# DataZooDE/anofox-forecast

Measured on AMD Instinct MI355X. Metric: series/sec fit+forecast, AutoETS h=28 on M5-shape batches, higher is better.
Workload: dtype f64

## Files before the change

anofox-forecast_amd/csrc/host_api.hip:

```cpp
#include <hip/hip_runtime.h>

#include <algorithm>
#include <cctype>
#include <atomic>
#include <memory>
#include <unordered_map>
#include <chrono>
#include <cmath>
#include <condition_variable>
#include <mutex>
#include <cstdio>
#include <cstdlib>
#include <cstring>
#include <limits>
#include <map>
#include <stdexcept>
#include <string>
#include <system_error>
#include <thread>
#include <vector>

#include "classic_device.hpp"
#include "host_semantics.hpp"
#include "kernels.hpp"
// ... 68 lines not shown
    int32_t *d_count = nullptr;
    int32_t *d_pos_map = nullptr, *d_pos_cnt = nullptr, *d_notpos = nullptr;
    double *d_ypos = nullptr;
    bool use_pos = false;
    bool none_pos = false;
    std::vector<anofox::FitArgs> insp_args;
    std::vector<anofox::FitLaunchers> insp_fns;
    std::vector<int> insp_spec, insp_stream;
    bool insp_ok = false;
    int insp_m = 1;
    int32_t live_pos = -1, live_all = -1;
    int arima_method = 0;
    size_t ar_ws_bytes = 0;
    double *ar_w = nullptr, *ar_wmean = nullptr, *ar_wsd = nullptr, *ar_l0 = nullptr, *ar_l1 = nullptr, *ar_x = nullptr, *ar_aicc = nullptr;
    int32_t *ar_wlen = nullptr, *ar_d = nullptr, *ar_D = nullptr, *ar_order = nullptr, *ar_status = nullptr, *ar_evals = nullptr, *ar_passes = nullptr, *ar_models = nullptr;
    StreamSet *sset = nullptr;
    hipStream_t own_stream = nullptr;
    hipStream_t aux[N_AUX_STREAMS] = {};
    hipEvent_t ev_start = nullptr, ev_stop = nullptr, ev_fit0 = nullptr, ev_fit1 = nullptr, ev_fork = nullptr;
    hipEvent_t ev_join[N_AUX_STREAMS] = {};
    struct Lane {
        double *ybuf = nullptr;
        size_t ybuf_cols = 0;
        int32_t *map[2] = {nullptr, nullptr};
        int32_t *cnt = nullptr;
        anofox::NmStateBuf st{};
        double *nm_scratch = nullptr;
        size_t nm_scratch_doubles = 0;
    } lanes[N_AUX_STREAMS];
    anofox::FitArgs *d_group_tab = nullptr, *h_group_tab = nullptr;
    size_t group_tab_cap = 0;
    hipEvent_t ev_group_tab = nullptr;
    hipStream_t last_stream = nullptr;
    bool ran = false, timed_fit = false;
    uint32_t fit_launches = 0;
    uint64_t n_problems = 0;
    Tunables tun;
    int seq_rounds = 3;
    int seq_rounds_env = -1;
    int spec_below_md = 8192;
    anofox::NmStateBuf classic_st{};
    int32_t *d_classic_status = nullptr, *classic_map[2] = {nullptr, nullptr}, *classic_cnt = nullptr;
    double *d_classic_ybuf = nullptr;
    size_t classic_ybuf_cols = 0;
    std::vector<void *> retired;
    int merged_m_max = 0;
    int32_t *d_m_col = nullptr;
    int spec2_below_md = 2048;
    int spec2_below = 1024;
    int spec_below = 8192;
    bool use_gather = false;
    double gather_budget = 0.0;
// ... 144 lines not shown
    if (b->owns_y) F(b->d_y);
    pin_free(b->h_stage);
    if (b->owns_len) F(b->d_len);
    F(b->d_mean); F(b->d_sd); F(b->d_fig_add); F(b->d_fig_mul); F(b->d_l0); F(b->d_b0); F(b->d_flags);
    F(b->d_aicc); F(b->d_yhat_slots); F(b->d_status_slots); F(b->d_evals_slots); F(b->d_iters_slots);
    F(b->d_passes_slots); F(b->d_slot_spec); F(b->d_lane_stats); F(b->d_wave_trace); F(b->d_yc32); F(b->d_yc16); F(b->d_misfit);
    F(b->d_yhat); F(b->d_lo); F(b->d_hi); F(b->d_model_code); F(b->d_status); F(b->d_detail);
    F(b->classic_st.sim); F(b->classic_st.fs); F(b->classic_st.phase); F(b->classic_st.evals); F(b->classic_st.iters); F(b->classic_st.passes); F(b->classic_st.done);
    F(b->d_classic_ybuf); F(b->d_classic_status); F(b->classic_map[0]); F(b->classic_map[1]); F(b->classic_cnt);
    for (void *p : b->retired) F(p);
    b->retired.clear();
    F(b->d_m_col); F(b->d_ring); F(b->d_prep_scratch);
    F(b->d_group_tab); pin_free(b->h_group_tab); b->d_group_tab = b->h_group_tab = nullptr; b->group_tab_cap = 0;
    if (b->ev_group_tab) { (void)hipEventDestroy(b->ev_group_tab); b->ev_group_tab = nullptr; }
    F(b->d_im_level); F(b->d_im_gmax); F(b->d_im_fc);
    F(b->d_th_sidx); F(b->d_th_adj);
    if (b->owns_exog) { F((void *)b->d_exog_x); F((void *)b->d_exog_f); }
    b->d_exog_x = b->d_exog_f = nullptr; b->owns_exog = false; b->exog_k = 0;
    F(b->d_exog_b0); F(b->d_exog_beta); F(b->d_exog_used);
    F(b->d_passes_total); F(b->d_evals_total); F(b->d_mask); F(b->d_len_group); F(b->d_count); F(b->d_pos_map); F(b->d_pos_cnt); F(b->d_notpos); F(b->d_ypos);
    F(b->ar_w); F(b->ar_wmean); F(b->ar_wsd); F(b->ar_l0); F(b->ar_l1); F(b->ar_x); F(b->ar_aicc); F(b->ar_wlen); F(b->ar_d); F(b->ar_D);
    F(b->ar_order); F(b->ar_status); F(b->ar_evals); F(b->ar_passes); F(b->ar_models);
    batch_detach_streams(b);
    for (auto &l : b->lanes) {
        F(l.ybuf); l.ybuf_cols = 0; F(l.map[0]); F(l.map[1]); F(l.cnt);
        F(l.st.sim); F(l.st.fs); F(l.st.phase); F(l.st.evals); F(l.st.iters); F(l.st.passes); F(l.st.done);
        F(l.nm_scratch); l.nm_scratch_doubles = 0;
    }
}

int max_slots_for(const Plan &p)
{
    if (p.model == M_AutoETS) return 30;
    if (p.model == M_ETS && p.ets_spec_id >= 0) return 1;
    return 0;
}

void alloc_common(AnofoxHipBatch *b)
{
    const size_t n = b->n, ld = b->ld, h = (size_t)std::max(b->h, 0);
    b->d_mean = dalloc<double>(ld);
    b->d_sd = dalloc<double>(ld);
    b->d_flags = dalloc<uint32_t>(ld);
    b->d_yhat = dalloc<double>(n * h);
    b->d_lo = dalloc<double>(n * h);
    b->d_hi = dalloc<double>(n * h);
    b->d_model_code = dalloc<int32_t>(ld);
    b->d_status = dalloc<int32_t>(ld);
// ... 22 lines not shown
        b->ar_status = dalloc<int32_t>(ld); b->ar_evals = dalloc<int32_t>(ld); b->ar_passes = dalloc<int32_t>(ld); b->ar_models = dalloc<int32_t>(ld);
        HIPCHECK(hipMemset(b->ar_wlen, 0, ld * sizeof(int32_t)));
    }
    HIPCHECK(hipMemset(b->d_model_code, 0, ld * sizeof(int32_t)));
    HIPCHECK(hipMemset(b->d_detail, 0, ld * sizeof(int32_t)));
    HIPCHECK(hipMemset(b->d_passes_total, 0, ld * sizeof(int32_t)));
    HIPCHECK(hipMemset(b->d_evals_total, 0, ld * sizeof(int32_t)));
    HIPCHECK(hipMemset(b->d_mask, 0, ld * sizeof(uint32_t)));
    b->n_slots_cap = max_slots_for(b->plan);
    if (b->n_slots_cap > 0) {
        const size_t S = (size_t)b->n_slots_cap;
        b->d_l0 = dalloc<double>(9 * ld);
        b->d_b0 = dalloc<double>(9 * ld);
        b->d_aicc = dalloc<double>(S * ld);
        b->d_yhat_slots = dalloc<double>(S * n * h);
        b->d_status_slots = dalloc<int32_t>(S * ld);
        b->d_evals_slots = dalloc<int32_t>(S * ld);
        b->d_iters_slots = dalloc<int32_t>(S * ld);
        b->d_passes_slots = dalloc<int32_t>(S * ld);
        b->d_slot_spec = dalloc<int32_t>(S);
        b->d_lane_stats = dalloc<unsigned long long>(2 * S);
        HIPCHECK(hipMemset(b->d_lane_stats, 0, 2 * S * sizeof(unsigned long long)));
        const int n_lanes = std::min<int>(N_AUX_STREAMS, b->n_slots_cap);
        for (int q = 0; q < n_lanes; q++) {
            auto &l = b->lanes[q];
            l.map[0] = dalloc<int32_t>(ld);
            l.map[1] = dalloc<int32_t>(ld);
            l.cnt = dalloc<int32_t>(3);
            l.st.sim = dalloc<double>(20 * ld);
            l.st.fs = dalloc<double>(5 * ld);
            l.st.phase = dalloc<int32_t>(ld);
            l.st.evals = dalloc<int32_t>(ld);
            l.st.iters = dalloc<int32_t>(ld);
            l.st.passes = dalloc<int32_t>(ld);
            l.st.done = dalloc<int32_t>(ld);
        }
    }
    batch_attach_streams(b);
}

void ensure_fig(AnofoxHipBatch *b, int m)
{
    if (m <= b->fig_m) return;
    if (b->d_fig_add) b->retired.push_back(b->d_fig_add);
    if (b->d_fig_mul) b->retired.push_back(b->d_fig_mul);
    b->d_fig_add = nullptr; b->d_fig_mul = nullptr; b->fig_m = 0;
    b->d_fig_add = dalloc<double>((size_t)m * b->ld);
    b->d_fig_mul = dalloc<double>((size_t)m * b->ld);
    b->fig_m = m;
}

// ... 146 lines not shown

void run_classic(AnofoxHipBatch *b, int kind, const int32_t *d_len, int m, int optimized, double alpha, int min_len,
                 const uint32_t *mask, uint32_t want, int32_t code, bool write_code, hipStream_t st)
{
    ClassicArgs a{};
    a.y = b->d_y; a.ld = b->ld; a.len = d_len; a.n_series = (int)b->n;
    a.m = m; a.h = b->h; a.optimized = optimized; a.fixed_alpha = alpha;
    a.mask = mask; a.want = want; a.min_len = min_len;
    a.yhat = b->d_yhat; a.status = b->d_detail; a.passes = b->d_passes_total;
    a.model_code = code; a.model_code_out = write_code ? b->d_model_code : nullptr;
    a.ring_scratch = nullptr;
    a.m_col = (kind == CK_HW || kind == CK_SEASONAL_ES) ? b->d_m_col : nullptr;
    const bool optimise = kind == CK_HOLT || kind == CK_HW || optimized != 0;
    if (optimise) {
        const size_t n = b->n, ld = b->ld;
        if (!b->classic_st.sim) {
            b->classic_st.sim = dalloc<double>(12 * ld); b->classic_st.fs = dalloc<double>(4 * ld);
            b->classic_st.phase = dalloc<int32_t>(ld); b->classic_st.evals = dalloc<int32_t>(ld); b->classic_st.iters = dalloc<int32_t>(ld);
            b->classic_st.passes = dalloc<int32_t>(ld); b->classic_st.done = dalloc<int32_t>(ld);
            b->d_classic_status = dalloc<int32_t>(ld);
            b->classic_map[0] = dalloc<int32_t>(ld); b->classic_map[1] = dalloc<int32_t>(ld); b->classic_cnt = dalloc<int32_t>(3);
        }
        double *ybuf = (b->n_slots_cap > 0 && b->use_gather) ? b->lanes[0].ybuf : nullptr;
        size_t ybuf_cols = ybuf ? b->lanes[0].ybuf_cols : ld;
        if (!ybuf) {
            const double per_col = (double)std::max<size_t>(b->t_max, 1) * 8.0;
            const size_t cols = (size_t)std::min((double)ld, 32.0 * 1073741824.0 / per_col) / 64 * 64;
            if (cols >= 1024 || cols >= ld) {
                if (!b->d_classic_ybuf) { b->d_classic_ybuf = dalloc<double>(std::max<size_t>(b->t_max, 1) * cols); b->classic_ybuf_cols = cols; }
                ybuf = b->d_classic_ybuf;
                ybuf_cols = b->classic_ybuf_cols;
            }
        }
        const bool seasonal = kind == CK_HW || kind == CK_SEASONAL_ES;
        FitArgs f{};
        f.y = b->d_y; f.ld = ld; f.len = d_len; f.n_series = (int)n; f.t_rows = (int)std::max<size_t>(b->t_max, 1);
        f.m = seasonal ? std::max(m, 1) : 1; f.h = b->h;
        f.flags = b->d_flags; f.fig = nullptr; f.fig_ld = ld;
        f.status = b->d_classic_status; f.st = b->classic_st;
        f.mask = mask; f.want = want; f.min_len = min_len;
        f.m_col = a.m_col;
        const bool merged = f.m_col != nullptr;
        FitLaunchers fns = classic_fit_launcher(kind, (merged && f.m == 7) ? 8 : f.m);
        if (!fns.round_seq || !fns.round_spec || !fns.round_spec2 || !fns.round_auto) throw HipFail{"no round kernel for this model"};
        if (f.m > ETS_LDS_PERIOD) {
            const size_t wg = merged ? n : std::max<size_t>((n + 15) / 16, std::min<size_t>(n, 1024));
            f.ring_scratch = ensure_ring(b, wg * (size_t)f.m * 64u);
// ... 319 lines not shown
            live_of[oi] = (spec_has_mult(specs[order[oi]]) && b->live_pos >= 0) ? (int64_t)b->live_pos : (b->live_all >= 0 ? (int64_t)b->live_all : (int64_t)n);
            lanes += live_of[oi];
        }
        const int64_t resident = 2 * 1024 * 64;
        const bool tiny_batch = (uint64_t)n * order.size() <= (uint64_t)TINY_BATCH_PROBLEMS;
        fill_mode = b->tun.fill_policy > 0 && !tiny_batch && !b->fixed_params && order.size() > 1 && b->seq_rounds_env < 0 && b->seq_rounds == 0 &&
                    lanes * 4 > 8 * resident;
        if (fill_mode) {
            const int64_t target = resident * (int64_t)b->tun.fill_target / 100;
            for (size_t oi = 0; oi < order.size(); oi++) {
                if (dead[oi] || k4[oi]) continue;
                if (lanes + 3 * live_of[oi] <= target) { fill_spec4[oi] = 1; lanes += 3 * live_of[oi]; }
            }
        }
    }
    if (b->use_gather && !b->fixed_params) {
        const size_t T = std::max<size_t>(b->t_max, 1);
        std::vector<size_t> need(order.size(), 0);
        double total = 0.0;
        for (size_t oi = 0; oi < order.size(); oi++) {
            if (dead[oi]) continue;
            size_t c = (b->use_pos && args[oi].need_positive && b->live_pos >= 0) ? (size_t)b->live_pos : n;
            need[oi] = std::min(ld, (c + 63) / 64 * 64);
            total += (double)need[oi] * (double)T * 8.0;
        }
        const double scale = total > b->gather_budget ? b->gather_budget / total : 1.0;
        for (size_t oi = 0; oi < order.size(); oi++) {
            if (dead[oi]) continue;
            auto &lane = b->lanes[oi % (size_t)n_lanes];
            size_t cols = scale < 1.0 ? (size_t)((double)need[oi] * scale) / 64 * 64 : need[oi];
            if (b->tun.gather_cols > 0) cols = std::min<size_t>(need[oi], (size_t)b->tun.gather_cols / 64 * 64);
            if (cols < need[oi] && cols < 1024 && b->tun.gather_cols <= 0) cols = 0;
            if (lane.ybuf && lane.ybuf_cols >= cols) continue;
            if (lane.ybuf) {
                HIPCHECK(hipDeviceSynchronize());
                dev_free(lane.ybuf, true);
                lane.ybuf = nullptr; lane.ybuf_cols = 0;
            }
            while (cols >= 64) {
                try { lane.ybuf = dalloc<double>(T * cols); lane.ybuf_cols = cols; break; }
                catch (const HipFail &f) {
                    if (!f.oom) throw;
                    cols = cols / 2 / 64 * 64;
                    if (cols < 1024) cols = 0;
                }
            }
        }
    }
    const bool tiny = (uint64_t)n * order.size() <= (uint64_t)TINY_BATCH_PROBLEMS;
    const int total_rounds = b->fixed_params ? 0 : (tiny ? 1 : n_rounds);
    enum { RK_SEQ, RK_SPEC, RK_SPEC2, RK_AUTO, RK_K4, RK_AUTO_K4 };
    std::vector<int> group_of(order.size(), -1);
    std::vector<std::vector<size_t>> groups;
    std::vector<int> group_stream;
    std::vector<GroupLaunchFn> group_fn;
    std::vector<size_t> slot_of(order.size(), 0);
    size_t n_slots = 0;
    bool grouped = b->tun.group_launch > 0 && !inline_stream && !tiny && !merged && !b->fixed_params && total_rounds > 0;
    if (grouped) {
        GroupLaunchFn fn[N_GROUP_CLASSES];
        for (int c = 0; c < N_GROUP_CLASSES; c++) fn[c] = ets_group_launcher(c, m, yt);
        std::vector<size_t> of_class[N_GROUP_CLASSES];
        for (size_t oi = 0; oi < order.size() && grouped; oi++) {
// ... 17 lines not shown
                }
                add(half[0], c); add(half[1], c);
            };
            if (b->tun.group_split == 1) add_split(of_class[GROUP_DAMPED_MUL], GROUP_DAMPED_MUL);
            else add(of_class[GROUP_DAMPED_MUL], GROUP_DAMPED_MUL);
            if (b->tun.group_split == 2) add_split(of_class[GROUP_GENERAL], GROUP_GENERAL);
            else add(of_class[GROUP_GENERAL], GROUP_GENERAL);
            add(of_class[GROUP_ADDITIVE], GROUP_ADDITIVE);
            grouped = !groups.empty();
        }
        if (grouped) {
            for (size_t g = 0; g < groups.size(); g++) {
                const bool dm = spec_trend_idx(specs[order[groups[g][0]]]) == 4;
                group_stream.push_back(dm ? (int)g : N_AUX_STREAMS - 1 - (int)g);
                for (size_t oi : groups[g]) { group_of[oi] = (int)g; stream_of[oi] = group_stream[g]; slot_of[oi] = n_slots++; }
            }
            for (size_t oi = 0; oi < order.size(); oi++) if (dead[oi]) stream_of[oi] = group_stream[0];
        }
    }
    bool emit = true;
    std::vector<int> slot_blocks, slot_k4;
    GroupCompactArgs gc{};
    GroupGatherArgs gg{};
    int gg_cols = 0;
    auto run_round = [&](const size_t oi, const int kind, const FitArgs &a, hipStream_t sq, const int r) {
        if (!grouped) {
            const FitLaunchFn f = kind == RK_SEQ ? fns[oi].round_seq : kind == RK_SPEC ? fns[oi].round_spec : kind == RK_SPEC2 ? fns[oi].round_spec2 :
                                  kind == RK_AUTO ? fns[oi].round_auto : kind == RK_K4 ? fns[oi].round_k4 : fns[oi].round_auto_k4;
            f(a, sq);
            return;
        }
        if (emit) return;
        FitArgs t = a;
        if (kind == RK_SEQ || kind == RK_K4) { t.spec_below = -1; t.spec2_below = -1; t.budget_seq = t.budget; }
        else if (kind == RK_SPEC) { t.spec_below = 0x7fffffff; t.spec2_below = -1; }
        else if (kind == RK_SPEC2) throw HipFail{"launch_fit_slots: the one-wave-per-problem round of a tiny batch has no group form"};
        const int g_seq = (int)((n + NM_BLOCK - 1) / NM_BLOCK);
        const int g_spec = (int)((std::min<int64_t>((int64_t)n, std::max(t.spec_below, 0)) + NM_BLOCK / NM_K - 1) / (NM_BLOCK / NM_K));
        const int g_spec2 = (int)std::min<int64_t>((int64_t)n, std::max(t.spec2_below, 0));
        const int blocks = std::max(g_seq, std::max(g_spec, g_spec2));
        if (t.ring_scratch != nullptr && (size_t)blocks * (size_t)t.m * NM_BLOCK > t.ring_scratch_doubles)
            throw HipFail{"launch_fit_slots: the seasonal-ring scratch does not cover a group slot"};
        const size_t cell = (size_t)r * n_slots + slot_of[oi];
        b->h_group_tab[cell] = t;
        slot_blocks[cell] = blocks;
        slot_k4[cell] = (kind == RK_K4 || kind == RK_AUTO_K4) ? 1 : 0;
// ... 11 lines not shown
            a.spec_below = -1; a.spec2_below = -1;
            a.gathered = 0;
            if (tiny) {
                a.y_round = b->d_y; a.ld_round = ld; a.series_of = nullptr; a.n_active = nullptr;
                a.budget = 1 << 30; a.budget_seq = a.budget;
                run_round(oi, RK_SPEC2, a, sq, r);
                b->fit_launches++;
                return;
            }
            if (r == 0 && b->use_pos && a.need_positive) {
                if (emit)
                    hipLaunchKernelGGL(retire_nonpositive_kernel, dim3((unsigned)((n + 255) / 256)), dim3(256), 0, sq, (int)n, d_len, b->d_notpos,
                                       a.status, lane.st.done, lane.st.passes, lane.st.evals, lane.st.iters);
                a.series_of = b->d_pos_map; a.n_active = b->d_pos_cnt;
                if (b->d_ypos) { a.y_round = b->d_ypos; a.ld_round = ld; a.gathered = 1; a.gather_cap = (int)ld; }
                else { a.y_round = b->d_y; a.ld_round = ld; }
            } else if (r == 0) {
                a.y_round = a.y; a.ld_round = ld; a.series_of = nullptr; a.n_active = nullptr;
            } else {
                const int32_t *prev_map = (r == 1) ? nullptr : lane.map[(r - 1) & 1];
                const int32_t *prev_cnt = (r == 1) ? nullptr : lane.cnt + ((r - 1) % 3);
                if (emit && !grouped && r == 1) HIPCHECK(hipMemsetAsync(lane.cnt, 0, 3 * sizeof(int32_t), sq));
                if (emit && !grouped) launch_compact(prev_map, prev_cnt, (int)n, lane.st.done, lane.map[r & 1], lane.cnt + (r % 3), sq, lane.cnt + ((r + 1) % 3));
                if (emit && grouped) {
                    const int k = gc.n_slots++;
                    gc.prev[k] = prev_map; gc.n_prev[k] = prev_cnt; gc.done[k] = lane.st.done;
                    gc.next[k] = lane.map[r & 1]; gc.n_next[k] = lane.cnt + (r % 3); gc.n_clear[k] = lane.cnt + ((r + 1) % 3);
                }
                a.series_of = lane.map[r & 1]; a.n_active = lane.cnt + (r % 3);
                if (b->use_gather && lane.ybuf) {
                    if (emit && !grouped)
                        launch_gather_columns(a.y, ld, lane.map[r & 1], lane.cnt + (r % 3), (int)n, (int)b->t_max, lane.ybuf, lane.ybuf_cols, sq,
                                              (int)lane.ybuf_cols, ybytes);
                    if (emit && grouped) {
                        const int k = gg.n_slots++;
                        gg.series_of[k] = lane.map[r & 1]; gg.n_active[k] = lane.cnt + (r % 3);
                        gg.out[k] = lane.ybuf; gg.ld_out[k] = lane.ybuf_cols; gg.cap[k] = (int)lane.ybuf_cols;
                        gg_cols = std::max(gg_cols, (int)std::min<size_t>(n, lane.ybuf_cols));
                    }
                    a.y_round = lane.ybuf; a.ld_round = lane.ybuf_cols; a.gathered = 1; a.gather_cap = (int)lane.ybuf_cols;
                } else {
                    a.y_round = a.y; a.ld_round = ld;
                }
            }
            const int s2 = (spec_trend_idx(specs[order[oi]]) == 4) ? b->spec2_below_md : b->spec2_below;
            if (fill_mode && !k4[oi]) {
                const int64_t live_i = (spec_has_mult(specs[order[oi]]) && b->live_pos >= 0) ? (int64_t)b->live_pos : (b->live_all >= 0 ? (int64_t)b->live_all : (int64_t)n);
                const int s2v = (int)std::max<int64_t>(32, std::min<int64_t>(s2 > 0 ? s2 : 32, live_i / std::max(1, b->tun.fill_s2_div)));
                a.budget = BUDGET[r]; a.budget_seq = (BUDGET[r] * 7) / 4;
                if (r == 0) {
                    if (fill_spec4[oi]) run_round(oi, RK_SPEC, a, sq, r);
                    else { a.budget = a.budget_seq; run_round(oi, RK_SEQ, a, sq, r); }
                } else {
                    a.spec_below = fill_spec4[oi] ? 0x7fffffff : (int)std::max<int64_t>(64, live_i / std::max(1, b->tun.fill_late_div));
                    a.spec2_below = s2v;
                    run_round(oi, RK_AUTO, a, sq, r);
                }
// ... 27 lines not shown
                a.budget = BUDGET[r];
                run_round(oi, RK_AUTO, a, sq, r);
            }
            if (!grouped) b->fit_launches++;
    };
    if (grouped) {
        const size_t cells = (size_t)total_rounds * n_slots;
        if (b->ev_group_tab) HIPCHECK(hipEventSynchronize(b->ev_group_tab));
        else HIPCHECK(hipEventCreateWithFlags(&b->ev_group_tab, hipEventDisableTiming));
        if (b->group_tab_cap < cells) {
            if (b->d_group_tab) b->retired.push_back(b->d_group_tab);
            pin_free(b->h_group_tab);
            b->d_group_tab = nullptr; b->h_group_tab = nullptr; b->group_tab_cap = 0;
            b->d_group_tab = dalloc<FitArgs>(cells);
            b->h_group_tab = (FitArgs *)pin_alloc_bytes(cells * sizeof(FitArgs));
            b->group_tab_cap = cells;
        }
        slot_blocks.assign(cells, 0); slot_k4.assign(cells, 0);
        emit = false;
        for (int r = 0; r < total_rounds; r++) for (size_t oi = 0; oi < order.size(); oi++) enqueue_round(r, oi);
        emit = true;
        HIPCHECK(hipMemcpyAsync(b->d_group_tab, b->h_group_tab, cells * sizeof(FitArgs), hipMemcpyHostToDevice, st));
        HIPCHECK(hipEventRecord(b->ev_group_tab, st));
        HIPCHECK(hipEventRecord(b->ev_fork, st));
        for (int q : group_stream) HIPCHECK(hipStreamWaitEvent(b->aux[q], b->ev_fork, 0));
    } else
        for (int i = 0; i < n_fork; i++) HIPCHECK(hipStreamWaitEvent(b->aux[i], b->ev_fit0, 0));
    for (size_t oi = 0; oi < order.size(); oi++)
        if (dead[oi]) {
            const FitArgs &a = args[oi];
            hipLaunchKernelGGL(retire_nonpositive_kernel, dim3((unsigned)((n + 255) / 256)), dim3(256), 0, spec_stream(stream_of[oi]), (int)n, d_len,
                               b->d_notpos, a.status, a.st.done, a.st.passes, a.st.evals, a.st.iters, a.aicc, a.passes, a.evals, a.iters);
        }
    if (b->fixed_params) {
        for (size_t oi = 0; oi < order.size(); oi++) {
            const int id = specs[order[oi]];
            FitArgs &a = args[oi];
            double x[4] = {0.0, 0.0, 0.0, 0.0};
            int d = 0;
            x[d++] = b->fixed_x[0];
            if (spec_trend_idx(id) != 0) x[d++] = b->fixed_x[1];
            if (spec_season(id) != 0) x[d++] = b->fixed_x[2];
            if (spec_trend_idx(id) == 2 || spec_trend_idx(id) == 4) x[d++] = b->fixed_x[3];
            hipLaunchKernelGGL(ets_fixed_setup_kernel, dim3((unsigned)((n + 255) / 256)), dim3(256), 0, spec_stream(stream_of[oi]), (int)n, ld, d_len,
                               b->d_flags, spec_season(id) != 0 ? 1 : 0, a.m, a.n_param, a.need_positive, d, x[0], x[1], x[2], x[3], a.status,
                               a.st.sim, a.st.evals, a.st.iters, a.st.passes, a.st.done);
        }
        LAUNCHCHECK("ETS fixed-parameter setup");
    }
    auto enqueue_group_round = [&](const int r, const size_t g) {
        hipStream_t sg = b->aux[group_stream[g]];
        if (r == 0) {
            int32_t *zero[GROUP_MAX_SLOTS] = {};
            for (size_t k = 0; k < groups[g].size(); k++) zero[k] = b->lanes[groups[g][k] % (size_t)n_lanes].cnt;
            launch_group_zero3((int)groups[g].size(), zero, sg);
        }
        gc = GroupCompactArgs{}; gc.n_series = (int)n;
        gg = GroupGatherArgs{}; gg.t_max = (int)b->t_max; gg.elem_bytes = ybytes; gg.y = ybase; gg.ld = ld; gg_cols = 0;
        for (size_t oi : groups[g]) enqueue_round(r, oi);
        if (gc.n_slots > 0) launch_group_compact(gc, sg);
        if (gg.n_slots > 0) launch_group_gather(gg, gg_cols, sg);
        GroupRoundArgs ga{};
        ga.n_slots = (int)groups[g].size();
        const size_t row = (size_t)r * n_slots + slot_of[groups[g][0]];
        for (int k = 0; k < ga.n_slots; k++) {
            const size_t oi = groups[g][(size_t)k];
            ga.spec[k] = specs[order[oi]];
            ga.k4[k] = slot_k4[(size_t)r * n_slots + slot_of[oi]];
            ga.start[k + 1] = ga.start[k] + slot_blocks[(size_t)r * n_slots + slot_of[oi]];
        }
        group_fn[g](b->d_group_tab + row, ga, m, sg);
        b->fit_launches++;
    };
    int head = 0;
    if (grouped && total_rounds > 0 && b->tun.dm_head_rounds > 0 && groups.size() > 1 && group_stream[0] == 0 &&
        spec_trend_idx(specs[order[groups[0][0]]]) == 4) {
        head = std::min(b->tun.dm_head_rounds, total_rounds);
        for (int r = 0; r < head; r++) enqueue_group_round(r, 0);
        LAUNCHCHECK("ETS fit head rounds");
        HIPCHECK(hipEventRecord(b->ev_join[0], b->aux[0]));
        for (size_t g = 1; g < groups.size(); g++) HIPCHECK(hipStreamWaitEvent(b->aux[group_stream[g]], b->ev_join[0], 0));
    } else if (!grouped && !tiny && !inline_stream && total_rounds > 0 && b->tun.dm_head_rounds > 0) {
// ... 3583 lines not shown
```

anofox-forecast_amd/csrc/host_resources.hpp:

```cpp
#pragma once

constexpr int N_AUX_STREAMS = 32;

struct HipFail { std::string msg; bool oom = false; };
void report_hip_failure(AnofoxError *out_error, const HipFail &f)
{
    if (f.oom) anofox::set_error(out_error, ALLOCATION_ERROR, "Allocation error: " + f.msg);
    else anofox::set_error(out_error, INTERNAL_ERROR, "Internal error: " + f.msg);
}
#define HIPCHECK(expr)                                                                             \
    do {                                                                                           \
        hipError_t _e = (expr);                                                                    \
        if (_e != hipSuccess) throw HipFail{std::string(#expr) + ": " + hipGetErrorString(_e), _e == hipErrorOutOfMemory};    \
    } while (0)

#define LAUNCHCHECK(what)                                                                          \
    do {                                                                                           \
        hipError_t _e = hipGetLastError();                                                         \
        if (_e != hipSuccess) throw HipFail{std::string("kernel launch failed (") + (what) + "): " + hipGetErrorString(_e), false};    \
    } while (0)

constexpr int32_t STATUS_NOT_COMPUTED = -1;

struct Tunables {
    std::vector<int> budgets{24, 24, 24, 24, 24, 24, 48, 48, 96, 96, 192, 1024};
    int seq_rounds = -1;
    int gather_cols = 0;
    int gather = -1;
    int spec_below = 8192;
    int spec_below_md = 8192;
    int spec2_below = 1024;
    int spec2_below_md = 2048;
    int k4 = -1;
    int k4_top = 1, k4_top_below = 20480;
    std::string wave_trace;
    int compact = -1;
    int fill_policy = 1;
    int fill_target = 150;
    int fill_late_div = 2;
    int fill_s2_div = 16;
    int top_boost_n = 0, top_boost_pct = 200;
    int prio_top = 0;
    int group_launch = 1;
    int group_split = 1;
    int dm_head_rounds = 0;
    bool merge_periods = true;
    int part_threads = 16;
    int pack_threads = 0;
    bool timing = false;
    int arima_trace = 0;
    double arima_lookahead = 6.0;
    int arima_lookahead_depth = 2;
    double arima_spec_factor = 4.0;
    double arima_shared_chunk_rounds = 1.0;
    int arima_prep_lanes = 64;
    int arima_queue_sort = 1;
    int arima_refit_budget = 100;
    static std::map<std::string, std::string> tune_map()
    {
        std::map<std::string, std::string> kv;
        const char *e = std::getenv("ANOFOX_HIP_TUNE");
        if (!e) return kv;
        std::string all(e);
        for (size_t pos = 0; pos < all.size();) {
            size_t end = all.find(';', pos);
            if (end == std::string::npos) end = all.size();
            const std::string item = all.substr(pos, end - pos);
// ... 13 lines not shown
        Tunables t;
        const std::map<std::string, std::string> kv = tune_map();
        auto geti = [&](const char *k, int &v) { auto it = kv.find(k); if (it != kv.end()) v = std::atoi(it->second.c_str()); };
        auto getd = [&](const char *k, double &v) { auto it = kv.find(k); if (it != kv.end()) v = std::atof(it->second.c_str()); };
        if (kv.count("budgets")) {
            std::vector<int> v;
            for (const char *q = kv.at("budgets").c_str(); *q;) {
                char *end = nullptr;
                long x = std::strtol(q, &end, 10);
                if (end == q) break;
                if (x > 0) v.push_back((int)x);
                q = (*end == ',') ? end + 1 : end;
            }
            if (!v.empty()) t.budgets = v;
        }
        if (kv.count("wave_trace")) t.wave_trace = kv.at("wave_trace");
        geti("compact", t.compact); geti("prio_top", t.prio_top); geti("top_boost_n", t.top_boost_n); geti("top_boost_pct", t.top_boost_pct);
        geti("fill_policy", t.fill_policy); geti("fill_target", t.fill_target); geti("fill_late_div", t.fill_late_div); geti("fill_s2_div", t.fill_s2_div);
        geti("seq_rounds", t.seq_rounds);
        geti("gather", t.gather);
        if (kv.count("spec_below")) t.spec_below = t.spec_below_md = std::atoi(kv.at("spec_below").c_str());
        geti("spec_below_md", t.spec_below_md);
        geti("gather_cols", t.gather_cols);
        geti("group_launch", t.group_launch); geti("group_split", t.group_split);
        geti("k4", t.k4); geti("dm_head_rounds", t.dm_head_rounds); geti("k4_top", t.k4_top); geti("k4_top_below", t.k4_top_below);
        if (kv.count("spec2_below")) t.spec2_below = t.spec2_below_md = std::atoi(kv.at("spec2_below").c_str());
        geti("spec2_below_md", t.spec2_below_md);
        if (kv.count("merge_periods")) t.merge_periods = std::atoi(kv.at("merge_periods").c_str()) != 0;
        geti("part_threads", t.part_threads);
        if (kv.count("arima_trace")) t.arima_trace = std::atoi(kv.at("arima_trace").c_str());
        getd("arima_lookahead", t.arima_lookahead);
        geti("arima_lookahead_depth", t.arima_lookahead_depth);
        getd("arima_spec_factor", t.arima_spec_factor);
        geti("arima_queue_sort", t.arima_queue_sort);
        geti("arima_prep_lanes", t.arima_prep_lanes);
        getd("arima_shared_chunk_rounds", t.arima_shared_chunk_rounds);
        geti("arima_refit_budget", t.arima_refit_budget);
        if (const char *e = std::getenv("ANOFOX_HIP_PACK_THREADS")) t.pack_threads = std::max(1, std::atoi(e));
        t.timing = std::getenv("ANOFOX_HIP_TIMING") != nullptr;
        return t;
    }
};
struct ProcessTunables {
    double cache_gb = -1.0, pinned_cache_gb = 2.0;
    double coalesce_us = 1000.0;
    int prio_streams = -1;
    std::string devices;
// ... 436 lines not shown
```

anofox-forecast_amd/csrc/kernels.hip:

```cpp
#include "classic_device.hpp"
#include "fit_units.hpp"
#include "kernels.hpp"

namespace anofox {

__global__ __launch_bounds__(NM_BLOCK) void select_kernel(const SelectArgs a)
{
    const int s = blockIdx.x * NM_BLOCK + threadIdx.x;
    if (s >= a.n_series) return;
    if (a.len[s] <= 0) { a.fallback_mask[s] = 0u; return; }
    int best = -1;
    double best_aicc = __builtin_huge_val();
    int passes = 0, evals = 0;
    for (int k = 0; k < a.n_slots; k++) {
        passes += a.passes_slots[(size_t)k * a.ld + s];
        evals += a.evals_slots[(size_t)k * a.ld + s];
        if (a.status_slots[(size_t)k * a.ld + s] != FIT_OK) continue;
        double v = a.aicc[(size_t)k * a.ld + s];
        if (v < best_aicc) { best_aicc = v; best = k; }
    }
    a.passes_total[s] = passes;
    a.evals_total[s] = evals;
    if (best < 0) {
        a.status[s] = -1;
// ... 282 lines not shown
        bool keep = false;
        if (idx < n_prev) {
            s = prev ? prev[idx] : idx;
            keep = done[s] == 0;
        }
        const unsigned long long bal = __ballot(keep);
        const int cnt = __popcll(bal);
        if (cnt == 0) continue;
        int base = 0;
        if (lane == 0) base = atomicAdd(g.n_next[k], cnt);
        base = __shfl(base, 0);
        const int before = __popcll(bal & ((1ull << lane) - 1ull));
        if (keep) g.next[k][base + before] = s;
    }
}

void launch_group_compact(const GroupCompactArgs &g, hipStream_t stream)
{
    if (g.n_slots <= 0 || g.n_series <= 0) return;
    const int grid = std::min((g.n_series + NM_BLOCK - 1) / NM_BLOCK, GROUP_COMPACT_BLOCKS);
    hipLaunchKernelGGL(group_compact_kernel, dim3(grid, g.n_slots), dim3(NM_BLOCK), 0, stream, g);
}

struct GroupZeroArgs { int32_t *p[GROUP_MAX_SLOTS]; };
__global__ void group_zero3_kernel(const int n, const GroupZeroArgs z)
{
    const int i = threadIdx.x;
    if (i < 3 * n) z.p[i / 3][i % 3] = 0;
}

void launch_group_zero3(int n, int32_t *const *zero, hipStream_t stream)
{
    if (n <= 0) return;
    GroupZeroArgs z{};
    for (int k = 0; k < n && k < GROUP_MAX_SLOTS; k++) z.p[k] = zero[k];
    hipLaunchKernelGGL(group_zero3_kernel, dim3(1), dim3(64), 0, stream, std::min(n, GROUP_MAX_SLOTS), z);
}

template <class E>
__global__ __launch_bounds__(NM_BLOCK) void group_gather_kernel(const GroupGatherArgs g)
{
    const int k = blockIdx.z;
    const int n_act = *g.n_active[k];
    if (n_act > g.cap[k]) return;
    const E *y = (const E *)g.y;
    E *out = (E *)g.out[k];
    const size_t ld_out = g.ld_out[k];
    const int32_t *series_of = g.series_of[k];
    for (int p0 = (int)blockIdx.x * NM_BLOCK; p0 < n_act; p0 += (int)gridDim.x * NM_BLOCK) {
        const int p = p0 + (int)threadIdx.x;
        const int s = series_of[p < n_act ? p : n_act - 1];
        for (int t0 = (int)blockIdx.y * GATHER_TB; t0 < g.t_max; t0 += (int)gridDim.y * GATHER_TB) {
            const int t1 = t0 + GATHER_TB < g.t_max ? t0 + GATHER_TB : g.t_max;
            for (int t = t0; t < t1; t++) out[(size_t)t * ld_out + p] = y[(size_t)t * g.ld + s];
        }
    }
}

void launch_group_gather(const GroupGatherArgs &g, int n_cols_max, hipStream_t stream)
{
    if (g.n_slots <= 0 || g.t_max <= 0 || n_cols_max <= 0) return;
    dim3 grid(std::min((n_cols_max + NM_BLOCK - 1) / NM_BLOCK, GROUP_GATHER_COL_BLOCKS),
              std::min((g.t_max + GATHER_TB - 1) / GATHER_TB, GROUP_GATHER_ROW_BLOCKS), g.n_slots);
    if (g.elem_bytes == 8) hipLaunchKernelGGL(group_gather_kernel<double>, grid, dim3(NM_BLOCK), 0, stream, g);
    else if (g.elem_bytes == 4) hipLaunchKernelGGL(group_gather_kernel<float>, grid, dim3(NM_BLOCK), 0, stream, g);
    else hipLaunchKernelGGL(group_gather_kernel<unsigned short>, grid, dim3(NM_BLOCK), 0, stream, g);
}

__global__ __launch_bounds__(NM_BLOCK) void compact_block_kernel(const double *y, size_t ld, const int32_t *len, int n_series, int t_rows, float *out32,
                                                                 unsigned short *out16, unsigned int *misfit)
{
    const int s = blockIdx.x * NM_BLOCK + threadIdx.x;
    const int t0 = blockIdx.y * GATHER_TB;
    const int t1 = t0 + GATHER_TB < t_rows ? t0 + GATHER_TB : t_rows;
    const int L = s < n_series ? len[s] : 0;
    unsigned bad32 = 0, bad16 = 0;
    if ((size_t)s < ld) {
        for (int t = t0; t < t1; t++) {
            const double v = y[(size_t)t * ld + s];
            const float f = (float)v;
            const unsigned short u = (v >= 0.0 && v <= 65535.0) ? (unsigned short)v : (unsigned short)0;
            out32[(size_t)t * ld + s] = f;
            if (out16) out16[(size_t)t * ld + s] = u;
            if (t < L) {
                bad32 += (__double_as_longlong((double)f) == __double_as_longlong(v)) ? 0u : 1u;
                bad16 += (__double_as_longlong((double)u) == __double_as_longlong(v)) ? 0u : 1u;
            }
        }
    }
// ... 134 lines not shown
```

anofox-forecast_amd/csrc/kernels.hpp:

```cpp
#pragma once
#include <hip/hip_runtime.h>
#include <stddef.h>
#include <stdint.h>
#include <atomic>

#include <stdexcept>
#include <string>

namespace anofox {

inline void anofox_check_attr(hipError_t e)
{
    if (e != hipSuccess) throw std::runtime_error(std::string("launch preparation failed: ") + hipGetErrorString(e));
}

enum : uint32_t { SF_POSITIVE = 1u, SF_CONSTANT = 2u, SF_HAS_NAN = 4u };

enum : int32_t { FIT_OK = 0, FIT_SHORT = 1, FIT_NONPOSITIVE = 2, FIT_NONFINITE = 3, FIT_PERIOD = 4, FIT_SKIPPED = 5 };

struct PrepArgs {
    const double *y; size_t ld; const int32_t *len; int n_series;
    int m;
    const int32_t *m_col;
    double *mean, *sd;
// ... 280 lines not shown
    int spec[GROUP_MAX_SLOTS];
    int k4[GROUP_MAX_SLOTS];
    int start[GROUP_MAX_SLOTS + 1];
};
typedef void (*GroupLaunchFn)(const FitArgs *tab, const GroupRoundArgs &g, int m, hipStream_t);
GroupLaunchFn ets_group_launcher(int group_class, int m, int yt);
inline int ets_group_class(int spec_id)
{
    if (spec_id < 0 || spec_id >= 30 || (spec_id >= 15 && spec_id % 3 == 1)) return -1;
    const int e = spec_id / 15, ti = (spec_id % 15) / 3, s = spec_id % 3;
    if (ti == 4) return GROUP_DAMPED_MUL;
    return (e == 0 && ti < 3 && s < 2) ? GROUP_ADDITIVE : GROUP_GENERAL;
}
FitLaunchers classic_fit_launcher(int kind, int m);
struct ClassicArgs;
void launch_classic_final(int kind, const FitArgs &a, const ClassicArgs &c, hipStream_t stream);

struct GroupCompactArgs {
    int n_slots, n_series;
    const int32_t *prev[GROUP_MAX_SLOTS], *n_prev[GROUP_MAX_SLOTS], *done[GROUP_MAX_SLOTS];
    int32_t *next[GROUP_MAX_SLOTS], *n_next[GROUP_MAX_SLOTS], *n_clear[GROUP_MAX_SLOTS];
};
void launch_group_compact(const GroupCompactArgs &g, hipStream_t);
void launch_group_zero3(int n, int32_t *const *zero, hipStream_t);
struct GroupGatherArgs {
    int n_slots, t_max, elem_bytes;
    const void *y; size_t ld;
    const int32_t *series_of[GROUP_MAX_SLOTS], *n_active[GROUP_MAX_SLOTS];
    void *out[GROUP_MAX_SLOTS]; size_t ld_out[GROUP_MAX_SLOTS]; int cap[GROUP_MAX_SLOTS];
};
void launch_group_gather(const GroupGatherArgs &g, int n_cols_max, hipStream_t);
void launch_compact(const int32_t *series_prev, const int32_t *n_prev, int n_series, const int32_t *done,
                    int32_t *series_next, int32_t *n_next, hipStream_t, int32_t *n_clear = nullptr);
constexpr int DETECT_LDS_ROWS = 8192;
constexpr int DETECT_LONG_GRID = 1024;
size_t detect_scratch_doubles(int n_series, int t_rows);
void launch_detect_periods(const double *y, size_t ld, const int32_t *len, int n_series, int t_rows, double *scratch, int32_t *period,
                           double *best_acf, hipStream_t stream);
void launch_gather_columns(const void *y, size_t ld, const int32_t *series_of, const int32_t *n_active, int n_series,
                           int t_max, void *out, size_t ld_out, hipStream_t stream, int cap, int elem_bytes = 8);
void launch_compact_block(const double *y, size_t ld, const int32_t *len, int n_series, int t_rows, float *out32, unsigned short *out16,
                          unsigned int *misfit, hipStream_t stream);

struct ArimaArgs {
    const double *y; size_t ld; const int32_t *len; int n_series;
    int m, h;
    int t_max;
    void *ws; size_t ws_bytes;
    int32_t *wlen, *d, *D;
    double *wmean, *wsd, *last_d0, *last_d1;
    int32_t *order;
    double *xbest;
    double *aicc;
    int32_t *status, *evals, *passes, *models;
// ... 29 lines not shown
```

Measured before the change: 79560.

## Add fused regroup kernel for compaction and gather, pool lane counters

Adds a group_regroup kernel that compacts surviving series with a wave ballot and gathers their columns into the lane buffer in the same launch, in place of separate compact and gather launches. It sits behind a tunable that defaults off. Per-lane counters move into one pooled allocation that is cleared with a single memset, replacing the per-group zero kernel launch. Lane buffers are now sized in bytes so narrower element types can reuse larger allocations.

Result: no change. 80050 (median of 2 runs) (+0.6%).

```diff
diff --git a/anofox-forecast_amd/csrc/host_api.hip b/anofox-forecast_amd/csrc/host_api.hip
--- a/anofox-forecast_amd/csrc/host_api.hip
+++ b/anofox-forecast_amd/csrc/host_api.hip
@@ -114,12 +114,14 @@
     struct Lane {
         double *ybuf = nullptr;
         size_t ybuf_cols = 0;
+        size_t ybuf_bytes = 0;
         int32_t *map[2] = {nullptr, nullptr};
         int32_t *cnt = nullptr;
         anofox::NmStateBuf st{};
         double *nm_scratch = nullptr;
         size_t nm_scratch_doubles = 0;
     } lanes[N_AUX_STREAMS];
+    int32_t *cnt_pool = nullptr;
     anofox::FitArgs *d_group_tab = nullptr, *h_group_tab = nullptr;
     size_t group_tab_cap = 0;
     hipEvent_t ev_group_tab = nullptr;
@@ -310,8 +312,9 @@
     F(b->ar_w); F(b->ar_wmean); F(b->ar_wsd); F(b->ar_l0); F(b->ar_l1); F(b->ar_x); F(b->ar_aicc); F(b->ar_wlen); F(b->ar_d); F(b->ar_D);
     F(b->ar_order); F(b->ar_status); F(b->ar_evals); F(b->ar_passes); F(b->ar_models);
     batch_detach_streams(b);
+    F(b->cnt_pool); b->cnt_pool = nullptr;
     for (auto &l : b->lanes) {
-        F(l.ybuf); l.ybuf_cols = 0; F(l.map[0]); F(l.map[1]); F(l.cnt);
+        F(l.ybuf); l.ybuf_cols = 0; l.ybuf_bytes = 0; F(l.map[0]); F(l.map[1]); l.cnt = nullptr;
         F(l.st.sim); F(l.st.fs); F(l.st.phase); F(l.st.evals); F(l.st.iters); F(l.st.passes); F(l.st.done);
         F(l.nm_scratch); l.nm_scratch_doubles = 0;
     }
@@ -380,11 +383,12 @@
         b->d_lane_stats = dalloc<unsigned long long>(2 * S);
         HIPCHECK(hipMemset(b->d_lane_stats, 0, 2 * S * sizeof(unsigned long long)));
         const int n_lanes = std::min<int>(N_AUX_STREAMS, b->n_slots_cap);
+        b->cnt_pool = dalloc<int32_t>(3 * (size_t)n_lanes);
         for (int q = 0; q < n_lanes; q++) {
             auto &l = b->lanes[q];
             l.map[0] = dalloc<int32_t>(ld);
             l.map[1] = dalloc<int32_t>(ld);
-            l.cnt = dalloc<int32_t>(3);
+            l.cnt = b->cnt_pool + 3 * q;
             l.st.sim = dalloc<double>(20 * ld);
             l.st.fs = dalloc<double>(5 * ld);
             l.st.phase = dalloc<int32_t>(ld);
@@ -577,7 +581,8 @@
             b->classic_map[0] = dalloc<int32_t>(ld); b->classic_map[1] = dalloc<int32_t>(ld); b->classic_cnt = dalloc<int32_t>(3);
         }
         double *ybuf = (b->n_slots_cap > 0 && b->use_gather) ? b->lanes[0].ybuf : nullptr;
-        size_t ybuf_cols = ybuf ? b->lanes[0].ybuf_cols : ld;
+        size_t ybuf_cols = ybuf ? std::min(ld, b->lanes[0].ybuf_bytes / (std::max<size_t>(b->t_max, 1) * sizeof(double)) / 64 * 64) : ld;
+        if (ybuf && ybuf_cols < 64) { ybuf = nullptr; ybuf_cols = ld; }
         if (!ybuf) {
             const double per_col = (double)std::max<size_t>(b->t_max, 1) * 8.0;
             const size_t cols = (size_t)std::min((double)ld, 32.0 * 1073741824.0 / per_col) / 64 * 64;
@@ -943,7 +948,7 @@
             if (dead[oi]) continue;
             size_t c = (b->use_pos && args[oi].need_positive && b->live_pos >= 0) ? (size_t)b->live_pos : n;
             need[oi] = std::min(ld, (c + 63) / 64 * 64);
-            total += (double)need[oi] * (double)T * 8.0;
+            total += (double)need[oi] * (double)T * (double)ybytes;
         }
         const double scale = total > b->gather_budget ? b->gather_budget / total : 1.0;
         for (size_t oi = 0; oi < order.size(); oi++) {
@@ -952,14 +957,17 @@
             size_t cols = scale < 1.0 ? (size_t)((double)need[oi] * scale) / 64 * 64 : need[oi];
             if (b->tun.gather_cols > 0) cols = std::min<size_t>(need[oi], (size_t)b->tun.gather_cols / 64 * 64);
             if (cols < need[oi] && cols < 1024 && b->tun.gather_cols <= 0) cols = 0;
-            if (lane.ybuf && lane.ybuf_cols >= cols) continue;
+            if (lane.ybuf && lane.ybuf_bytes >= T * cols * (size_t)ybytes) {
+                lane.ybuf_cols = std::min(ld, lane.ybuf_bytes / (T * (size_t)ybytes) / 64 * 64);
+                continue;
+            }
             if (lane.ybuf) {
                 HIPCHECK(hipDeviceSynchronize());
                 dev_free(lane.ybuf, true);
-                lane.ybuf = nullptr; lane.ybuf_cols = 0;
+                lane.ybuf = nullptr; lane.ybuf_cols = 0; lane.ybuf_bytes = 0;
             }
             while (cols >= 64) {
-                try { lane.ybuf = dalloc<double>(T * cols); lane.ybuf_cols = cols; break; }
+                try { lane.ybuf = (double *)dalloc<char>(T * cols * (size_t)ybytes); lane.ybuf_cols = cols; lane.ybuf_bytes = T * cols * (size_t)ybytes; break; }
                 catch (const HipFail &f) {
                     if (!f.oom) throw;
                     cols = cols / 2 / 64 * 64;
@@ -1023,6 +1031,7 @@
     std::vector<int> slot_blocks, slot_k4;
     GroupCompactArgs gc{};
     GroupGatherArgs gg{};
+    GroupRegroupArgs gr{};
     int gg_cols = 0;
     auto run_round = [&](const size_t oi, const int kind, const FitArgs &a, hipStream_t sq, const int r) {
         if (!grouped) {
@@ -1080,7 +1089,15 @@
                 const int32_t *prev_cnt = (r == 1) ? nullptr : lane.cnt + ((r - 1) % 3);
                 if (emit && !grouped && r == 1) HIPCHECK(hipMemsetAsync(lane.cnt, 0, 3 * sizeof(int32_t), sq));
                 if (emit && !grouped) launch_compact(prev_map, prev_cnt, (int)n, lane.st.done, lane.map[r & 1], lane.cnt + (r % 3), sq, lane.cnt + ((r + 1) % 3));
-                if (emit && grouped) {
+                const bool regroup = grouped && b->tun.group_regroup > 0 && b->use_gather && lane.ybuf;
+                if (emit && regroup) {
+                    const int k = gr.n_slots++;
+                    gr.prev[k] = prev_map; gr.n_prev[k] = prev_cnt; gr.done[k] = lane.st.done;
+                    gr.next[k] = lane.map[r & 1]; gr.n_next[k] = lane.cnt + (r % 3); gr.n_clear[k] = lane.cnt + ((r + 1) % 3);
+                    gr.out[k] = lane.ybuf; gr.ld_out[k] = lane.ybuf_cols; gr.cap[k] = (int)lane.ybuf_cols;
+                    gr.out_elems[k] = lane.ybuf_bytes / (size_t)ybytes;
+                }
+                if (emit && grouped && !regroup) {
                     const int k = gc.n_slots++;
                     gc.prev[k] = prev_map; gc.n_prev[k] = prev_cnt; gc.done[k] = lane.st.done;
                     gc.next[k] = lane.map[r & 1]; gc.n_next[k] = lane.cnt + (r % 3); gc.n_clear[k] = lane.cnt + ((r + 1) % 3);
@@ -1090,7 +1107,7 @@
                     if (emit && !grouped)
                         launch_gather_columns(a.y, ld, lane.map[r & 1], lane.cnt + (r % 3), (int)n, (int)b->t_max, lane.ybuf, lane.ybuf_cols, sq,
                                               (int)lane.ybuf_cols, ybytes);
-                    if (emit && grouped) {
+                    if (emit && grouped && !regroup) {
                         const int k = gg.n_slots++;
                         gg.series_of[k] = lane.map[r & 1]; gg.n_active[k] = lane.cnt + (r % 3);
                         gg.out[k] = lane.ybuf; gg.ld_out[k] = lane.ybuf_cols; gg.cap[k] = (int)lane.ybuf_cols;
@@ -1164,6 +1181,7 @@
         emit = true;
         HIPCHECK(hipMemcpyAsync(b->d_group_tab, b->h_group_tab, cells * sizeof(FitArgs), hipMemcpyHostToDevice, st));
         HIPCHECK(hipEventRecord(b->ev_group_tab, st));
+        HIPCHECK(hipMemsetAsync(b->cnt_pool, 0, 3 * (size_t)n_lanes * sizeof(int32_t), st));
         HIPCHECK(hipEventRecord(b->ev_fork, st));
         for (int q : group_stream) HIPCHECK(hipStreamWaitEvent(b->aux[q], b->ev_fork, 0));
     } else
@@ -1192,14 +1210,11 @@
     }
     auto enqueue_group_round = [&](const int r, const size_t g) {
         hipStream_t sg = b->aux[group_stream[g]];
-        if (r == 0) {
-            int32_t *zero[GROUP_MAX_SLOTS] = {};
-            for (size_t k = 0; k < groups[g].size(); k++) zero[k] = b->lanes[groups[g][k] % (size_t)n_lanes].cnt;
-            launch_group_zero3((int)groups[g].size(), zero, sg);
-        }
         gc = GroupCompactArgs{}; gc.n_series = (int)n;
         gg = GroupGatherArgs{}; gg.t_max = (int)b->t_max; gg.elem_bytes = ybytes; gg.y = ybase; gg.ld = ld; gg_cols = 0;
+        gr = GroupRegroupArgs{}; gr.n_series = (int)n; gr.t_max = (int)b->t_max; gr.elem_bytes = ybytes; gr.y = ybase; gr.ld = ld;
         for (size_t oi : groups[g]) enqueue_round(r, oi);
+        if (gr.n_slots > 0) launch_group_regroup(gr, sg);
         if (gc.n_slots > 0) launch_group_compact(gc, sg);
         if (gg.n_slots > 0) launch_group_gather(gg, gg_cols, sg);
         GroupRoundArgs ga{};
diff --git a/anofox-forecast_amd/csrc/host_resources.hpp b/anofox-forecast_amd/csrc/host_resources.hpp
--- a/anofox-forecast_amd/csrc/host_resources.hpp
+++ b/anofox-forecast_amd/csrc/host_resources.hpp
@@ -43,6 +43,7 @@
     int prio_top = 0;
     int group_launch = 1;
     int group_split = 1;
+    int group_regroup = 0;
     int dm_head_rounds = 0;
     bool merge_periods = true;
     int part_threads = 16;
@@ -102,7 +103,7 @@
         if (kv.count("spec_below")) t.spec_below = t.spec_below_md = std::atoi(kv.at("spec_below").c_str());
         geti("spec_below_md", t.spec_below_md);
         geti("gather_cols", t.gather_cols);
-        geti("group_launch", t.group_launch); geti("group_split", t.group_split);
+        geti("group_launch", t.group_launch); geti("group_split", t.group_split); geti("group_regroup", t.group_regroup);
         geti("k4", t.k4); geti("dm_head_rounds", t.dm_head_rounds); geti("k4_top", t.k4_top); geti("k4_top_below", t.k4_top_below);
         if (kv.count("spec2_below")) t.spec2_below = t.spec2_below_md = std::atoi(kv.at("spec2_below").c_str());
         geti("spec2_below_md", t.spec2_below_md);
diff --git a/anofox-forecast_amd/csrc/kernels.hip b/anofox-forecast_amd/csrc/kernels.hip
--- a/anofox-forecast_amd/csrc/kernels.hip
+++ b/anofox-forecast_amd/csrc/kernels.hip
@@ -328,21 +328,6 @@
     hipLaunchKernelGGL(group_compact_kernel, dim3(grid, g.n_slots), dim3(NM_BLOCK), 0, stream, g);
 }
 
-struct GroupZeroArgs { int32_t *p[GROUP_MAX_SLOTS]; };
-__global__ void group_zero3_kernel(const int n, const GroupZeroArgs z)
-{
-    const int i = threadIdx.x;
-    if (i < 3 * n) z.p[i / 3][i % 3] = 0;
-}
-
-void launch_group_zero3(int n, int32_t *const *zero, hipStream_t stream)
-{
-    if (n <= 0) return;
-    GroupZeroArgs z{};
-    for (int k = 0; k < n && k < GROUP_MAX_SLOTS; k++) z.p[k] = zero[k];
-    hipLaunchKernelGGL(group_zero3_kernel, dim3(1), dim3(64), 0, stream, std::min(n, GROUP_MAX_SLOTS), z);
-}
-
 template <class E>
 __global__ __launch_bounds__(NM_BLOCK) void group_gather_kernel(const GroupGatherArgs g)
 {
@@ -371,6 +356,77 @@
     if (g.elem_bytes == 8) hipLaunchKernelGGL(group_gather_kernel<double>, grid, dim3(NM_BLOCK), 0, stream, g);
     else if (g.elem_bytes == 4) hipLaunchKernelGGL(group_gather_kernel<float>, grid, dim3(NM_BLOCK), 0, stream, g);
     else hipLaunchKernelGGL(group_gather_kernel<unsigned short>, grid, dim3(NM_BLOCK), 0, stream, g);
+}
+
+#ifndef ANOFOX_REGROUP_WAVES
+#define ANOFOX_REGROUP_WAVES 4
+#endif
+constexpr int REGROUP_WAVES = ANOFOX_REGROUP_WAVES, REGROUP_TB = 16, GROUP_REGROUP_BLOCKS = 256;
+template <class E>
+__global__ __launch_bounds__(NM_BLOCK * REGROUP_WAVES) void group_regroup_kernel(const GroupRegroupArgs g)
+{
+    __shared__ int sh_series[NM_BLOCK];
+    __shared__ int sh_base, sh_cnt;
+    const int k = blockIdx.y;
+    if (g.n_clear[k] && blockIdx.x == 0 && threadIdx.x == 0) *g.n_clear[k] = 0;
+    const int n_prev = g.n_prev[k] ? *g.n_prev[k] : g.n_series;
+    const int32_t *prev = g.prev[k], *done = g.done[k];
+    const E *y = (const E *)g.y;
+    E *out = (E *)g.out[k];
+    const size_t ld = g.ld, ld_out = g.ld_out[k];
+    const int cap = g.cap[k], t_max = g.t_max;
+    const int lane = threadIdx.x & (NM_BLOCK - 1), wave = threadIdx.x / NM_BLOCK;
+    for (int base0 = (int)blockIdx.x * NM_BLOCK; base0 < n_prev; base0 += (int)gridDim.x * NM_BLOCK) {
+        if (wave == 0) {
+            const int idx = base0 + lane;
+            int s = 0;
+            bool keep = false;
+            if (idx < n_prev) {
+                s = prev ? prev[idx] : idx;
+                keep = done[s] == 0;
+            }
+            const unsigned long long bal = __ballot(keep);
+            const int cnt = __popcll(bal);
+            int base = 0;
+            if (cnt > 0) {
+                if (lane == 0) base = atomicAdd(g.n_next[k], cnt);
+                base = __shfl(base, 0);
+                const int before = __popcll(bal & ((1ull << lane) - 1ull));
+                if (keep) { g.next[k][base + before] = s; sh_series[before] = s; }
+            }
+            if (lane == 0) { sh_base = base; sh_cnt = cnt; }
+        }
+        __syncthreads();
+        const int p = sh_base + lane;
+        if (lane < sh_cnt && p < cap) {
+            const E *src = y + sh_series[lane];
+            E *dst = out + p;
+            for (int t0 = wave * REGROUP_TB; t0 < t_max; t0 += REGROUP_WAVES * REGROUP_TB) {
+                if (t0 + REGROUP_TB <= t_max) {
+                    E v[REGROUP_TB];
+#pragma unroll
+                    for (int i = 0; i < REGROUP_TB; i++) v[i] = src[(size_t)(t0 + i) * ld];
+#pragma unroll
+                    for (int i = 0; i < REGROUP_TB; i++) dst[(size_t)(t0 + i) * ld_out] = v[i];
+                } else
+                    for (int t = t0; t < t_max; t++) dst[(size_t)t * ld_out] = src[(size_t)t * ld];
+            }
+        }
+        __syncthreads();
+    }
+}
+
+void launch_group_regroup(const GroupRegroupArgs &g, hipStream_t stream)
+{
+    if (g.n_slots <= 0 || g.n_series <= 0) return;
+    if (g.n_slots > GROUP_MAX_SLOTS) throw std::runtime_error("launch_group_regroup: more slots than GROUP_MAX_SLOTS");
+    for (int k = 0; k < g.n_slots; k++)
+        if (g.cap[k] < 0 || (size_t)g.cap[k] > g.ld_out[k] || (size_t)std::max(g.t_max, 0) * g.ld_out[k] > g.out_elems[k])
+            throw std::runtime_error("launch_group_regroup: the gather block does not cover a group slot");
+    const dim3 grid(std::min((g.n_series + NM_BLOCK - 1) / NM_BLOCK, GROUP_REGROUP_BLOCKS), g.n_slots), block(NM_BLOCK * REGROUP_WAVES);
+    if (g.elem_bytes == 8) hipLaunchKernelGGL(group_regroup_kernel<double>, grid, block, 0, stream, g);
+    else if (g.elem_bytes == 4) hipLaunchKernelGGL(group_regroup_kernel<float>, grid, block, 0, stream, g);
+    else hipLaunchKernelGGL(group_regroup_kernel<unsigned short>, grid, block, 0, stream, g);
 }
 
 __global__ __launch_bounds__(NM_BLOCK) void compact_block_kernel(const double *y, size_t ld, const int32_t *len, int n_series, int t_rows, float *out32,
diff --git a/anofox-forecast_amd/csrc/kernels.hpp b/anofox-forecast_amd/csrc/kernels.hpp
--- a/anofox-forecast_amd/csrc/kernels.hpp
+++ b/anofox-forecast_amd/csrc/kernels.hpp
@@ -326,7 +326,6 @@
     int32_t *next[GROUP_MAX_SLOTS], *n_next[GROUP_MAX_SLOTS], *n_clear[GROUP_MAX_SLOTS];
 };
 void launch_group_compact(const GroupCompactArgs &g, hipStream_t);
-void launch_group_zero3(int n, int32_t *const *zero, hipStream_t);
 struct GroupGatherArgs {
     int n_slots, t_max, elem_bytes;
     const void *y; size_t ld;
@@ -334,6 +333,14 @@
     void *out[GROUP_MAX_SLOTS]; size_t ld_out[GROUP_MAX_SLOTS]; int cap[GROUP_MAX_SLOTS];
 };
 void launch_group_gather(const GroupGatherArgs &g, int n_cols_max, hipStream_t);
+struct GroupRegroupArgs {
+    int n_slots, n_series, t_max, elem_bytes;
+    const void *y; size_t ld;
+    const int32_t *prev[GROUP_MAX_SLOTS], *n_prev[GROUP_MAX_SLOTS], *done[GROUP_MAX_SLOTS];
+    int32_t *next[GROUP_MAX_SLOTS], *n_next[GROUP_MAX_SLOTS], *n_clear[GROUP_MAX_SLOTS];
+    void *out[GROUP_MAX_SLOTS]; size_t ld_out[GROUP_MAX_SLOTS], out_elems[GROUP_MAX_SLOTS]; int cap[GROUP_MAX_SLOTS];
+};
+void launch_group_regroup(const GroupRegroupArgs &g, hipStream_t);
 void launch_compact(const int32_t *series_prev, const int32_t *n_prev, int n_series, const int32_t *done,
                     int32_t *series_next, int32_t *n_next, hipStream_t, int32_t *n_clear = nullptr);
 constexpr int DETECT_LDS_ROWS = 8192;
```
